# ViacheslavDanilov/oct_segmentation

Hardware: AMD Instinct MI355X
Metric: OCT frames/sec (704x704, bf16) fwd+bwd (higher is better)
Workload: dtype bf16; 1 GPU; unetplusplus/resnet101 1-class 704x704, batch 16/GPU, fwd+Dice+bwd+allreduce+Adam; global_batch=16, parallelism=dp1

## Files before the change

### oct_segmentation_amd/csrc/conv_mfma.hip

```cpp
#include "common.h"
#include "conv_common.h"
#include "kernels.h"

#include <type_traits>

namespace octseg {

#ifdef OCTSEG_STAMP
#define STAMP(var) do { __builtin_amdgcn_sched_barrier(0); asm volatile("s_memtime %0\n\ts_waitcnt lgkmcnt(0)" : "=s"(var) :: "memory"); __builtin_amdgcn_sched_barrier(0); } while (0)
#else
#define STAMP(var) do { } while (0)
#endif

struct RowMap {
  static constexpr unsigned MASK_B = 0xF00F0FF0u;
  static __device__ __forceinline__ int ty(int rr) { return (MASK_B >> rr) & 1; }
  static __device__ __forceinline__ int tx(int rr) {
    const unsigned grp = ((MASK_B >> rr) & 1) ? MASK_B : ~MASK_B;
    return __popc(grp & ((1u << rr) - 1u));
  }
};

static constexpr int wave_mt(int NT, int RB) { return (NT == 4 && RB == 64) ? 4 : 2; }

// ... 271 lines not shown
          const int gy = y0 + ty, gx = x0 + tx;
          float val = acc16[mb][nb][j] + bias;
          if (a.relu_out) val = clamp_lo(val, 0.f);
          if (cok && pv && gy < a.OH && gx < a.OW) {
            s1[nb] += val; s2[nb] += val * val;
            if (head) {
              const DstDesc& d = a.dst[0];
              const int oy = gy * a.ostride + a.ooy, ox = gx * a.ostride + a.oox;
              ((float*)d.ptr)[(((size_t)n * a.Cout + co) * d.H + oy) * d.W + ox] = val;
            }
          }
          if (!head) *(unsigned short*)(otile + prow * OPITCH + cl * 2) = Tr<T>::bits16(val);
        }
    }
  } else
#pragma unroll
  for (int nt = 0; nt < NT; ++nt) {
    s1[nt] = 0.f; s2[nt] = 0.f;
    const int cl = wn * NT * 32 + nt * 32 + r;
    const int co = co0 + cl;
    const bool cok = co < a.Cout;
    const float bias = (a.bias != nullptr && cok) ? a.bias[co] : 0.f;
#pragma unroll
    for (int mt = 0; mt < MT; ++mt) {
#pragma unroll
      for (int i = 0; i < 16; ++i) {
        const int rr = (i & 3) + 8 * (i >> 2) + 4 * h;
        const int ty = wm * 2 * MT + mt * 2 + RowMap::ty(rr), tx = RowMap::tx(rr);
        const int gy = y0 + ty, gx = x0 + tx;
        float val = acc[mt][nt][i] + bias;
        if (a.relu_out) val = clamp_lo(val, 0.f);
        if (cok && gy < a.OH && gx < a.OW) {
          s1[nt] += val; s2[nt] += val * val;
          if (head) {
            const DstDesc& d = a.dst[0];
            const int oy = gy * a.ostride + a.ooy, ox = gx * a.ostride + a.oox;
            ((float*)d.ptr)[(((size_t)n * a.Cout + co) * d.H + oy) * d.W + ox] = val;
          }
        }
        if (!head) {
          if (sizeof(T) == 4) *(float*)(otile + (ty * TW + tx) * OPITCH + cl * 4) = val;
          else *(unsigned short*)(otile + (ty * TW + tx) * OPITCH + cl * 2) = Tr<T>::bits16(val);
        }
      }
    }
  }
  if (a.stat_slab != nullptr) {
    if constexpr (M16) {
#pragma unroll
      for (int nb = 0; nb < NCB; ++nb) {
        s1[nb] += __shfl_xor(s1[nb], 16); s1[nb] += __shfl_xor(s1[nb], 32);
        s2[nb] += __shfl_xor(s2[nb], 16); s2[nb] += __shfl_xor(s2[nb], 32);
        if (g16 == 0) {
          const int cl = wn * NT * 32 + nb * 16 + r16;
          red[(wm * BN + cl) * 2 + 0] = s1[nb];
          red[(wm * BN + cl) * 2 + 1] = s2[nb];
        }
      }
    } else
#pragma unroll
    for (int nt = 0; nt < NT; ++nt) {
      s1[nt] += __shfl_xor(s1[nt], 32);
      s2[nt] += __shfl_xor(s2[nt], 32);
      if (h == 0) {
        const int cl = wn * NT * 32 + nt * 32 + r;
        red[(wm * BN + cl) * 2 + 0] = s1[nt];
        red[(wm * BN + cl) * 2 + 1] = s2[nt];
      }
    }
  }
  __syncthreads();
  if (a.stat_slab != nullptr && tid < BN) {
    const int co = co0 + tid;
    if (co < a.Cout) {
      float t1 = 0.f, t2 = 0.f;
#pragma unroll
      for (int w = 0; w < WM; ++w) { t1 += red[(w * BN + tid) * 2]; t2 += red[(w * BN + tid) * 2 + 1]; }
      float* slab = a.stat_slab + ((size_t)(a.slab_row0 + (w_mt)) * a.Cout + co) * 2;
      slab[0] = t1; slab[1] = t2;
    }
  }
  if (!head) {
    for (int v = tid; v < BM * OVPR; v += NTHREADS) {
      const int p = v / OVPR, cvv = v % OVPR;
      int ty = p >> 4, tx = p & 15;
      if constexpr (T11) { if (p >= 121) continue; ty = p / 11; tx = p - ty * 11; }
      const int gy = y0 + ty, gx = x0 + tx;
      const int co = co0 + cvv * VEC;
      if (gy >= a.OH || gx >= a.OW || co >= a.Cout) continue;
      char* dptr = (char*)a.dst[0].ptr; int dC = a.dst[0].C, dc0 = a.dst[0].c0, dH = a.dst[0].H, dW = a.dst[0].W, dacc = a.dst[0].accum;
      int dpool = a.dst[0].pool;
#pragma unroll
      for (int i = 1; i < MAX_SRC; ++i)
        if (i < a.ndst && co >= a.dst[i].c0) {
          dptr = (char*)a.dst[i].ptr; dC = a.dst[i].C; dc0 = a.dst[i].c0; dH = a.dst[i].H; dW = a.dst[i].W; dacc = a.dst[i].accum;
          dpool = a.dst[i].pool;
        }
      if (dpool) {
        if ((ty | tx) & 1) continue;
        const char* l0 = otile + p * OPITCH + cvv * 16;
        const uint4 q[4] = {*(const uint4*)l0, *(const uint4*)(l0 + OPITCH), *(const uint4*)(l0 + TW * OPITCH),
                            *(const uint4*)(l0 + (TW + 1) * OPITCH)};
        uint4* gq = (uint4*)(dptr + ((((size_t)n * dH + (gy >> 1)) * dW + (gx >> 1)) * dC + (co - dc0)) * sizeof(T));
        uint4 old = make_uint4(0, 0, 0, 0);
        if (dacc) old = *gq;
        unsigned o[4] = {old.x, old.y, old.z, old.w}, r4[4];
        const unsigned* qq[4] = {&q[0].x, &q[1].x, &q[2].x, &q[3].x};
#pragma unroll
        for (int i = 0; i < 4; ++i) {
          if (sizeof(T) == 4) {
            float sacc = dacc ? __uint_as_float(o[i]) : 0.f;
#pragma unroll
            for (int j = 0; j < 4; ++j) sacc += __uint_as_float(qq[j][i]);
            r4[i] = __float_as_uint(sacc);
          } else {
            float lo = dacc ? Tr<T>::lo(o[i]) : 0.f, hi = dacc ? Tr<T>::hi(o[i]) : 0.f;
#pragma unroll
            for (int j = 0; j < 4; ++j) { lo += Tr<T>::lo(qq[j][i]); hi += Tr<T>::hi(qq[j][i]); }
            r4[i] = Tr<T>::pk(lo, hi);
          }
        }
        *gq = make_uint4(r4[0], r4[1], r4[2], r4[3]);
        continue;
      }
      const int oy = gy * a.ostride + a.ooy, ox = gx * a.ostride + a.oox;
      uint4* gp = (uint4*)(dptr + ((((size_t)n * dH + oy) * dW + ox) * dC + (co - dc0)) * sizeof(T));
      uint4 val = *(const uint4*)(otile + p * OPITCH + cvv * 16);
      if (a.out_mode == OUT_ACCUM || dacc) {
        const uint4 old = *gp;
        if (sizeof(T) == 4) {
          val.x = __float_as_uint(__uint_as_float(val.x) + __uint_as_float(old.x));
          val.y = __float_as_uint(__uint_as_float(val.y) + __uint_as_float(old.y));
          val.z = __float_as_uint(__uint_as_float(val.z) + __uint_as_float(old.z));
          val.w = __float_as_uint(__uint_as_float(val.w) + __uint_as_float(old.w));
        } else {
          unsigned nv[4] = {val.x, val.y, val.z, val.w};
          const unsigned ov[4] = {old.x, old.y, old.z, old.w};
#pragma unroll
          for (int i = 0; i < 4; ++i) {
            const float lo = Tr<T>::lo(nv[i]) + Tr<T>::lo(ov[i]);
            const float hi = Tr<T>::hi(nv[i]) + Tr<T>::hi(ov[i]);
            nv[i] = Tr<T>::pk(lo, hi);
          }
          val = make_uint4(nv[0], nv[1], nv[2], nv[3]);
        }
      }
      *gp = val;
    }
  }
}

template <int RB> struct ConvCfg { static constexpr int PITCH = RB + 16, KSTEPS = RB / 32, VPR = RB / 16; };

enum { LOOP_GENERIC = 0, LOOP_RESIDENT = 1, LOOP_1X1 = 2, LOOP_RUN9 = 3, LOOP_RUN9S = 4, LOOP_MASKED = 5, LOOP_T11 = 6, LOOP_MASKED_T11 = 7 };

template <typename T, int NT, int WN, int WM, int RB, int LOOP>
__global__ __launch_bounds__(64 * WM * WN, ((WM * WN == 4 && wave_mt(NT, RB) == 2) ? 2 : 1)) void conv_mfma_kernel(const ConvArgs a, const int mode) {
  constexpr int MT = wave_mt(NT, RB);
  const int dbuf = mode & 1;
  constexpr bool resident = LOOP == LOOP_RESIDENT;
  extern __shared__ __attribute__((aligned(16))) char smem[];
  constexpr int NTHREADS = 64 * WM * WN;
  constexpr int BN = NT * 32 * WN;
  constexpr int TH = 2 * MT * WM;
  constexpr int KC = RB / (int)sizeof(T);
  constexpr int PITCH = ConvCfg<RB>::PITCH, KSTEPS = ConvCfg<RB>::KSTEPS, VPR = ConvCfg<RB>::VPR;
  constexpr int NWAVES = WM * WN;
  constexpr int BBYTES = BN * RB;
  constexpr int NDMA = BBYTES / 1024;
  constexpr int DPW = (NDMA + NWAVES - 1) / NWAVES;
  constexpr int SWZ_DIV = 256 / RB;
  constexpr int MAXP = 4;
  typedef WindowStager<T, RB, NTHREADS> Stager;

#ifdef OCTSEG_STAMP
  unsigned long long k0 = 0, k1 = 0, k2 = 0, k3 = 0;
  STAMP(k0);
#endif
  const int tid = threadIdx.x, lane = tid & 63, wave = tid >> 6;
  const int wm = wave / WN, wn = wave % WN;
  const int r = lane & 31, h = lane >> 5;

  constexpr bool T11 = LOOP == LOOP_T11 || LOOP == LOOP_MASKED_T11;
  const TilePos tp = map_tile<TH, BN, T11>(a);
  const int n = tp.n, y0 = tp.y0, x0 = tp.x0, nt_idx = tp.nt_idx;

  const bool single = a.ntaps == 1;
  const int lstride = single ? 1 : a.istride;
  const int smul = single ? a.istride : 1;
  constexpr int THe = T11 ? 11 : TH, TWe = T11 ? 11 : TW;
  const int RH = single ? THe : (THe - 1) * a.istride + a.span_y;
  const int RW = single ? TWe : (TWe - 1) * a.istride + a.span_x;
  const int npix = RH * RW;
  const int npass = (npix + Stager::PSTEP - 1) / Stager::PSTEP;
  const float inv_rw = 1.0f / (float)RW;
  const int gy0 = y0 * a.istride + a.min_dy, gx0 = x0 * a.istride + a.min_dx;

  const int abytes = npass * Stager::PSTEP * PITCH;
  char* ldsA = smem;
  char* ldsB = smem + (dbuf ? 2 : 1) * abytes;

  constexpr bool M16 = conv_m16<T>(MT);
  f32x16_t acc[M16 ? 1 : MT][M16 ? 1 : NT];
#pragma unroll
  for (int i = 0; i < (M16 ? 1 : MT); ++i)
#pragma unroll
    for (int j = 0; j < (M16 ? 1 : NT); ++j)
#pragma unroll
      for (int k = 0; k < 16; ++k) acc[i][j][k] = 0.f;
  f32x4_t acc16[M16 ? 2 * MT : 1][M16 ? 2 * NT : 1];
#pragma unroll
  for (int i = 0; i < (M16 ? 2 * MT : 1); ++i)
#pragma unroll
    for (int j = 0; j < (M16 ? 2 * NT : 1); ++j)
#pragma unroll
      for (int k = 0; k < 4; ++k) acc16[i][j][k] = 0.f;
  const int r16 = lane & 15, g16 = lane >> 4;
  int abase16[2 * MT], bbase16[2 * NT], bswz16[2 * NT];
#pragma unroll
  for (int mb = 0; mb < 2 * MT; ++mb) {
    abase16[mb] = (((wm * 2 * MT + mb) * lstride) * RW + r16 * lstride) * PITCH + g16 * 16;
    if constexpr (T11) {
      const int p = min((wm * 2 * MT + mb) * 16 + r16, 120);
      const int pty = p / 11;
      abase16[mb] = (pty * RW + (p - pty * 11)) * PITCH + g16 * 16;
    }
  }
#pragma unroll
  for (int nb = 0; nb < 2 * NT; ++nb) {
    const int row = wn * NT * 32 + nb * 16 + r16;
    bbase16[nb] = row * RB;
    bswz16[nb] = (row / SWZ_DIV) & (VPR - 1);
  }

  int abase[MT], bbase[NT];
#pragma unroll
  for (int mt = 0; mt < MT; ++mt) {
    const int ty = wm * 2 * MT + mt * 2 + RowMap::ty(r), tx = RowMap::tx(r);
    abase[mt] = ((ty * lstride) * RW + tx * lstride) * PITCH + h * 16;
  }
  int bswz[NT];
#pragma unroll
  for (int nt = 0; nt < NT; ++nt) {
    const int row = wn * NT * 32 + nt * 32 + r;
    bbase[nt] = row * RB;
    bswz[nt] = (row / SWZ_DIV) & (VPR - 1);
  }

  const int nchunks = (a.Cin + KC - 1) / KC;
  const char* Wp = (const char*)a.W;

  const int ntiles_n = gridDim.y;
  const int wave_u = __builtin_amdgcn_readfirstlane(wave);
  const unsigned ldsB_addr = (unsigned)(size_t)(__attribute__((address_space(3))) char*)ldsB;
  const char* dma_src0 = Wp + (size_t)nt_idx * BBYTES + (size_t)wave_u * DPW * 1024 + lane * 16;
  const size_t slab_stride = (size_t)ntiles_n * BBYTES;
  const bool dma_wave = NDMA % NWAVES == 0 || wave_u * DPW < NDMA;
  auto dmaB = [&](int slab_idx, int slot) {
    if (dma_wave) {
      const char* gsrc0 = dma_src0 + (size_t)slab_idx * slab_stride;
#pragma unroll
      for (int j = 0; j < DPW; ++j) {
        const char* gsrc = gsrc0 + j * 1024;
        const unsigned dst = __builtin_amdgcn_readfirstlane(ldsB_addr + slot * BBYTES + (wave_u * DPW + j) * 1024);
        unsigned keep;
        asm volatile("s_mov_b32 %0, m0\n\ts_mov_b32 m0, %2\n\ts_nop 0\n\tglobal_load_lds_dwordx4 %1, off\n\ts_mov_b32 m0, %0"
                     : "=&s"(keep) : "v"(gsrc), "s"(dst) : "memory");
      }
    }
  };
  int v_toff = 0, v_tapw = 0;
  if (lane < a.ntaps) {
    v_toff = single ? 0 : ((a.tap_dy[lane] - a.min_dy) * RW + (a.tap_dx[lane] - a.min_dx)) * PITCH;
    v_tapw = a.tap_w[lane];
  }
  auto stage_full = [&](const Stager& sg, char* dst) {
    for (int p = 0; p < npass; p += MAXP) {
      uint4 v[MAXP];
      bool ok[MAXP];
#pragma unroll
      for (int u = 0; u < MAXP; ++u) v[u] = sg.load(min(p + u, npass - 1), n, gy0, gx0, smul, RW, npix, inv_rw, a.IH, a.IW, ok[u]);
#pragma unroll
      for (int u = 0; u < MAXP; ++u) sg.write(dst, min(p + u, npass - 1), v[u], ok[u]);
    }
  };
  auto mma_tap = [&](const char* awin, const char* bsl, int toff) {
    if constexpr (M16) {
      constexpr int KQ = RB / 64;
      uint4 fa[2 * MT], fb[KQ][2 * NT];
      auto ldA = [&](int mb, int kq) __attribute__((always_inline)) { fa[mb] = *(const uint4*)(awin + abase16[mb] + toff + kq * 64); };
      auto ldB = [&](int kq, int nb) __attribute__((always_inline)) {
        fb[kq][nb] = *(const uint4*)(bsl + bbase16[nb] + (((kq * 4 + g16) ^ bswz16[nb]) * 16));
      };
      ldA(0, 0);
#pragma unroll
      for (int nb = 0; nb < 2 * NT; ++nb) ldB(0, nb);
#pragma unroll
      for (int mb = 1; mb < 2 * MT; ++mb) ldA(mb, 0);
#pragma unroll
      for (int kq = 0; kq < KQ; ++kq)
#pragma unroll
        for (int mb = 0; mb < 2 * MT; ++mb) {
          __builtin_amdgcn_sched_barrier(0);
#pragma unroll
          for (int nb = 0; nb < 2 * NT; ++nb) Tr<T>::mma16(fa[mb], fb[kq][nb], acc16[mb][nb]);
          if (kq + 1 < KQ) {
            ldA(mb, kq + 1);
// ... 43 lines not shown
#pragma unroll
      for (int kq = 0; kq < KQ; ++kq)
#pragma unroll
        for (int mb = 0; mb < 2 * MT; ++mb) {
          __builtin_amdgcn_sched_barrier(0);
#pragma unroll
          for (int nb = 0; nb < 2 * NT; ++nb) Tr<T>::mma16(fa[mb], fb[kq][nb], acc16[mb][nb]);
          if (kq + 1 < KQ) {
            ldA(mb, kq + 1);
#pragma unroll
            for (int nb = 0; nb < 2 * NT; ++nb)
              if (nb * 2 * MT / (2 * NT) == mb) ldB(kq + 1, nb);
          }
          __builtin_amdgcn_sched_barrier(0);
          {
            constexpr int NSTEP = KQ * 2 * MT;
            const int step = kq * 2 * MT + mb;
            if (step == NSTEP / 4 - 1 || (NSTEP < 4 && step == 0)) f0();
            if (step == NSTEP / 2 - 1) f1();
            if (step == (3 * NSTEP) / 4 - 1 || (NSTEP < 4 && step == NSTEP - 1)) f2();
            __builtin_amdgcn_sched_barrier(0);
          }
        }
    } else {
    constexpr int NFB = KSTEPS >= 3 ? 3 : KSTEPS;
    uint4 af[NFB][MT], bf[NFB][NT];
    auto frag_load = [&](int buf, int ks) {
#pragma unroll
      for (int mt = 0; mt < MT; ++mt) af[buf][mt] = *(const uint4*)(awin + abase[mt] + toff + ks * 32);
#pragma unroll
      for (int nt = 0; nt < NT; ++nt) bf[buf][nt] = *(const uint4*)(bsl + bbase[nt] + (((ks * 2 + h) ^ bswz[nt]) * 16));
    };
    frag_load(0, 0);
    if (KSTEPS > 1) frag_load(1, 1);
#pragma unroll
    for (int ks = 0; ks < KSTEPS; ++ks) {
      if (ks + 2 < KSTEPS) frag_load((ks + 2) % NFB, ks + 2);
      __builtin_amdgcn_sched_barrier(0);
#pragma unroll
      for (int mt = 0; mt < MT; ++mt)
#pragma unroll
        for (int nt = 0; nt < NT; ++nt) Tr<T>::mma(af[ks % NFB][mt], bf[ks % NFB][nt], acc[mt][nt]);
      __builtin_amdgcn_sched_barrier(0);
      if (ks == 0) f0();
      if (ks == 1) f1();
      if (ks == 2 || (KSTEPS == 2 && ks == 1)) f2();
      __builtin_amdgcn_sched_barrier(0);
    }
    }
  };

  {
    Stager cur;
    cur.setup(a.src, a.nsrc, a.Cin, 0, tid);
    if (resident) {
      for (int t = 0; t < a.ntaps; ++t) dmaB(a.tap_w[t] * nchunks, t);
    } else if constexpr (LOOP == LOOP_MASKED || LOOP == LOOP_MASKED_T11) {
      dmaB(a.tap_w[a.src_taps[0] & 15] * nchunks, 0);
    } else {
      dmaB(a.tap_w[0] * nchunks, 0);
      if constexpr (LOOP == LOOP_RUN9 || LOOP == LOOP_RUN9S) dmaB(a.tap_w[1] * nchunks, 1);
    }
    stage_full(cur, ldsA);
  }
  asm volatile("s_waitcnt vmcnt(0)" ::: "memory");
  __syncthreads();
#ifdef OCTSEG_STAMP
  STAMP(k1);
#endif

#ifdef OCTSEG_STAMP
  unsigned long long tsum[6] = {0, 0, 0, 0, 0, 0};
#endif
  const int IHl = a.IH, IWl = a.IW, ntaps = a.ntaps;
  const int p0w = tid / VPR;
  const int hy_first = (int)(((float)p0w + 0.5f) * inv_rw), hx_first = p0w - hy_first * RW;
  const int dq = Stager::PSTEP / RW, dr = Stager::PSTEP - dq * RW;
  auto run = [&](auto ppt_c, auto dbuf_c) {
    constexpr int PPT = decltype(ppt_c)::value;
    constexpr bool DBUF = decltype(dbuf_c)::value;
    int it = 0;
    int tap2 = ntaps == 1 ? 0 : 1, chunk2 = ntaps == 1 ? min(1, nchunks - 1) : 0;
    for (int chunk = 0; chunk < nchunks; ++chunk) {
      const bool has_next = chunk + 1 < nchunks;
      Stager nxt;
      nxt.setup(a.src, a.nsrc, a.Cin, has_next ? chunk + 1 : chunk, tid, a.src_uniform != 0);
      nxt.bind_image(n);
      const char* awin = ldsA + ((DBUF && (chunk & 1)) ? abytes : 0);
      char* anext = ldsA + ((chunk & 1) ? 0 : abytes);
      int hy = hy_first, hx = hx_first, hp = p0w;
      char* wrow = anext + p0w * PITCH;
      for (int t = 0; t < ntaps; ++t, ++it) {
        unsigned long long s0 = 0, s1 = 0, s2 = 0, s3 = 0, s4 = 0, s5 = 0;
        (void)s0; (void)s1; (void)s2; (void)s3; (void)s4; (void)s5;
        STAMP(s0);
        uint4 av[PPT];
        bool aok[PPT];
        char* wr[PPT];
        if constexpr (DBUF) {
#pragma unroll
          for (int u = 0; u < PPT; ++u) {
            av[u] = nxt.load_at(hy, hx, hp < npix, gy0, gx0, smul, IHl, IWl, aok[u]);
            wr[u] = wrow;
            const bool adv = hp + Stager::PSTEP < npass * Stager::PSTEP;
            if (adv) {
              hp += Stager::PSTEP; wrow += Stager::PSTEP * PITCH;
              hy += dq; hx += dr;
              if (hx >= RW) { hx -= RW; hy += 1; }
            }
          }
        }
        dmaB(__builtin_amdgcn_readlane(v_tapw, tap2) * nchunks + chunk2, (it + 1) & 1);
        const int toff = __builtin_amdgcn_readlane(v_toff, t);
        STAMP(s1);
        mma_tap(awin, ldsB + (it & 1) * BBYTES, toff);
        STAMP(s2);
        __builtin_amdgcn_sched_barrier(0);
        if constexpr (DBUF) {
#pragma unroll
          for (int u = 0; u < PPT; ++u) nxt.write_at(wr[u], av[u], aok[u]);
        }
        STAMP(s3);
        asm volatile("s_waitcnt vmcnt(0)" ::: "memory");
        asm volatile("s_waitcnt lgkmcnt(0)" ::: "memory");
        STAMP(s4);
        __builtin_amdgcn_s_barrier();
        asm volatile("" ::: "memory");
        STAMP(s5);
#ifdef OCTSEG_STAMP
        tsum[0] += s1 - s0; tsum[1] += s2 - s1; tsum[2] += s3 - s2; tsum[3] += s4 - s3; tsum[4] += s5 - s4; tsum[5] += 1;
#endif
        if (++tap2 == ntaps) { tap2 = 0; chunk2 = min(chunk2 + 1, nchunks - 1); }
      }
      if constexpr (!DBUF) {
        if (has_next) {
          stage_full(nxt, ldsA);
          __syncthreads();
        }
      }
    }
  };
  auto run_t11 = [&](auto np_c) {
    constexpr int NP = decltype(np_c)::value;
    int it = 0;
    int tap2 = 1, chunk2 = 0;
    for (int chunk = 0; chunk < nchunks; ++chunk) {
      const bool has_next = chunk + 1 < nchunks;
      Stager nxt;
      nxt.setup(a.src, a.nsrc, a.Cin, has_next ? chunk + 1 : chunk, tid, a.src_uniform != 0);
      nxt.bind_image(n);
      uint4 av[NP];
      bool aok[NP];
      int hy = hy_first, hx = hx_first, hp = p0w;
#pragma unroll
      for (int t = 0; t < 9; ++t, ++it) {
        if (t < NP) {
          av[t] = nxt.load_at(hy, hx, hp < npix, gy0, gx0, smul, IHl, IWl, aok[t]);
          const bool adv = hp + Stager::PSTEP < npass * Stager::PSTEP;
          if (adv) {
            hp += Stager::PSTEP;
            hy += dq; hx += dr;
            if (hx >= RW) { hx -= RW; hy += 1; }
          }
        }
        dmaB(__builtin_amdgcn_readlane(v_tapw, tap2) * nchunks + chunk2, (it + 1) & 1);
        const int toff = __builtin_amdgcn_readlane(v_toff, t);
        mma_tap(ldsA, ldsB + (it & 1) * BBYTES, toff);
        __builtin_amdgcn_sched_barrier(0);
        asm volatile("s_waitcnt vmcnt(0)" ::: "memory");
        asm volatile("s_waitcnt lgkmcnt(0)" ::: "memory");
        __builtin_amdgcn_s_barrier();
        asm volatile("" ::: "memory");
        if (++tap2 == 9) { tap2 = 0; chunk2 = min(chunk2 + 1, nchunks - 1); }
      }
      if (has_next) {
#pragma unroll
        for (int u = 0; u < NP; ++u)
          if (u < npass) nxt.write_at(ldsA + (p0w + u * Stager::PSTEP) * PITCH, av[u], aok[u]);
        __syncthreads();
      }
    }
  };
  auto run_masked = [&](auto ppt_c) {
    constexpr int PPT = decltype(ppt_c)::value;
    const int tps = a.taps_per_src;
    auto list_of = [&](int chunk) -> int {
      int l = a.src_taps[0];
#pragma unroll
      for (int i = 1; i < MAX_SRC; ++i)
        if (i < a.nsrc && chunk * KC >= a.src[i].c0) l = a.src_taps[i];
      return l;
    };
    int it = 0;
    for (int chunk = 0; chunk < nchunks; ++chunk) {
      const bool has_next = chunk + 1 < nchunks;
      const int cnext = has_next ? chunk + 1 : chunk;
      Stager nxt;
      nxt.setup(a.src, a.nsrc, a.Cin, cnext, tid, a.src_uniform != 0);
      nxt.bind_image(n);
      const char* awin = ldsA + ((chunk & 1) ? abytes : 0);
      char* anext = ldsA + ((chunk & 1) ? 0 : abytes);
      const int lst = list_of(chunk), lst_n = list_of(cnext);
      int hy = hy_first, hx = hx_first, hp = p0w;
      char* wrow = anext + p0w * PITCH;
      for (int k = 0; k < tps; ++k, ++it) {
        const int t = (lst >> (4 * k)) & 15;
        uint4 av[PPT];
        bool aok[PPT];
        char* wr[PPT];
        const bool same = k + 1 < tps;
        const int tn = same ? (lst >> (4 * (k + 1))) & 15 : lst_n & 15;
        const int toff = __builtin_amdgcn_readlane(v_toff, t);
        mma_tap_f(awin, ldsB + (it & 1) * BBYTES, toff,
          [&]() {
            dmaB(__builtin_amdgcn_readlane(v_tapw, tn) * nchunks + (same ? chunk : cnext), (it + 1) & 1);
#pragma unroll
            for (int u = 0; u < PPT; ++u) {
              av[u] = nxt.load_at(hy, hx, hp < npix, gy0, gx0, smul, IHl, IWl, aok[u]);
              wr[u] = wrow;
              const bool adv = hp + Stager::PSTEP < npass * Stager::PSTEP;
              if (adv) {
                hp += Stager::PSTEP; wrow += Stager::PSTEP * PITCH;
                hy += dq; hx += dr;
                if (hx >= RW) { hx -= RW; hy += 1; }
              }
            }
          },
          [&]() {},
          [&]() {
#pragma unroll
            for (int u = 0; u < PPT; ++u) nxt.write_at(wr[u], av[u], aok[u]);
          });
        __builtin_amdgcn_sched_barrier(0);
        asm volatile("s_waitcnt vmcnt(0)" ::: "memory");
        asm volatile("s_waitcnt lgkmcnt(0)" ::: "memory");
        __builtin_amdgcn_s_barrier();
        asm volatile("" ::: "memory");
      }
    }
  };
  typedef __attribute__((ext_vector_type(4))) unsigned u32x4_t;
  auto run1p = [&]() __attribute__((always_inline)) {
    constexpr int PPT = 4;
    constexpr int NQ = 2 * (Stager::VEC / 4);
    constexpr int NLD = PPT + NQ;
    constexpr int NDM = NDMA % NWAVES == 0 ? DPW : 0;
    Stager sA, sB;
    u32x4_t avA0 = {0, 0, 0, 0}, avA1 = avA0, avA2 = avA0, avA3 = avA0, qA0 = avA0, qA1 = avA0, qA2 = avA0, qA3 = avA0;
    u32x4_t avB0 = avA0, avB1 = avA0, avB2 = avA0, avB3 = avA0, qB0 = avA0, qB1 = avA0, qB2 = avA0, qB3 = avA0;
    bool okA[PPT], okB[PPT];
    int pyc[PPT], pxc[PPT];
    bool pok[PPT];
    {
      int hy = hy_first, hx = hx_first, hp = p0w;
#pragma unroll
      for (int u = 0; u < PPT; ++u) {
        const int iy = gy0 + hy * smul, ix = gx0 + hx * smul;
        pok[u] = hp < npix && (unsigned)iy < (unsigned)IHl && (unsigned)ix < (unsigned)IWl;
        pyc[u] = min(max(iy, 0), IHl - 1); pxc[u] = min(max(ix, 0), IWl - 1);
        const bool adv = hp + Stager::PSTEP < npass * Stager::PSTEP;
        if (adv) {
          hp += Stager::PSTEP;
          hy += dq; hx += dr;
          if (hx >= RW) { hx -= RW; hy += 1; }
        }
      }
    }
    const bool usrc = a.src_uniform != 0;
#define OCTSEG_LD4(dst, ptr) asm volatile("global_load_dwordx4 %0, %1, off" : "=v"(dst) : "v"(ptr))
#define OCTSEG_LD4_16(dst, ptr) asm volatile("global_load_dwordx4 %0, %1, off offset:16" : "=v"(dst) : "v"(ptr))
    auto load_chunk = [&](Stager& sg, int chunk, u32x4_t& v0, u32x4_t& v1, u32x4_t& v2, u32x4_t& v3, u32x4_t& q0, u32x4_t& q1,
                          u32x4_t& q2, u32x4_t& q3, bool (&ok)[PPT]) __attribute__((always_inline)) {
      sg.select(a.src, a.nsrc, a.Cin, min(chunk, nchunks - 1), tid, usrc);
      sg.bind_image(n);
      const char* scp = sg.has_aff ? (const char*)(sg.s.scale + sg.s.cl) : Wp;
      const char* shp = sg.has_aff ? (const char*)(sg.s.shift + sg.s.cl) : Wp;
      OCTSEG_LD4(q0, scp);
      if constexpr (Stager::VEC == 8) OCTSEG_LD4_16(q1, scp);
      OCTSEG_LD4(q2, shp);
      if constexpr (Stager::VEC == 8) OCTSEG_LD4_16(q3, shp);
      const char* g0 = sg.addr_xy(pyc[0], pxc[0]); OCTSEG_LD4(v0, g0);
      const char* g1 = sg.addr_xy(pyc[1], pxc[1]); OCTSEG_LD4(v1, g1);
      const char* g2 = sg.addr_xy(pyc[2], pxc[2]); OCTSEG_LD4(v2, g2);
      const char* g3 = sg.addr_xy(pyc[3], pxc[3]); OCTSEG_LD4(v3, g3);
#pragma unroll
      for (int u = 0; u < PPT; ++u) ok[u] = sg.cvalid && pok[u];
    };
    auto body = [&](int c, Stager& sld, u32x4_t& l0, u32x4_t& l1, u32x4_t& l2, u32x4_t& l3, u32x4_t& lq0, u32x4_t& lq1, u32x4_t& lq2,
                    u32x4_t& lq3, bool (&okl)[PPT], Stager& sst, u32x4_t& s0, u32x4_t& s1, u32x4_t& s2, u32x4_t& s3, u32x4_t& sq0,
                    u32x4_t& sq1, u32x4_t& sq2, u32x4_t& sq3, const bool (&oks)[PPT]) __attribute__((always_inline)) {
      char* wnext = ldsA + ((c & 1) ? 0 : abytes);
      auto row = [&](int u) { return wnext + (min(u, npass - 1) * Stager::PSTEP + p0w) * PITCH; };
      mma_tap_f(ldsA + ((c & 1) ? abytes : 0), ldsB + (c & 1) * BBYTES, 0,
        [&]() {
          dmaB(a.tap_w[0] * nchunks + min(c + 1, nchunks - 1), (c + 1) & 1);
          load_chunk(sld, c + 2, l0, l1, l2, l3, lq0, lq1, lq2, lq3, okl);
        },
        [&]() {
          asm volatile("s_waitcnt vmcnt(%8)" : "+v"(s0), "+v"(s1), "+v"(s2), "+v"(s3), "+v"(sq0), "+v"(sq1), "+v"(sq2), "+v"(sq3)
                       : "n"(NDM + NLD) : "memory");
#pragma unroll
          for (int i = 0; i < 4; ++i) {
            sst.sc[i] = __uint_as_float(sq0[i]); sst.sh[i] = __uint_as_float(sq2[i]);
            if constexpr (Stager::VEC == 8) { sst.sc[4 + i] = __uint_as_float(sq1[i]); sst.sh[4 + i] = __uint_as_float(sq3[i]); }
          }
          sst.write_at(row(0), __builtin_bit_cast(uint4, s0), oks[0]);
          sst.write_at(row(1), __builtin_bit_cast(uint4, s1), oks[1]);
        },
        [&]() {
          sst.write_at(row(2), __builtin_bit_cast(uint4, s2), oks[2]);
// ... 71 lines not shown
                if (hx >= RW) { hx -= RW; hy += 1; }
              }
            }
          },
          [&]() {
            STAMP(s2);
            if constexpr (TT >= 1) {
              if constexpr ((TT - 1) & 1) {
                asm volatile("s_waitcnt vmcnt(%1)" : "+v"(avB) : "n"(DPW + W) : "memory");
                STAMP(s3);
                wv = nxt.prep(__builtin_bit_cast(uint4, avB), okB);
              } else {
                asm volatile("s_waitcnt vmcnt(%1)" : "+v"(avA) : "n"(DPW + W) : "memory");
                STAMP(s3);
                wv = nxt.prep(__builtin_bit_cast(uint4, avA), okA);
              }
            } else {
              asm volatile("s_waitcnt vmcnt(%4)" : "+v"(q0), "+v"(q1), "+v"(q2), "+v"(q3) : "n"(DPW + W) : "memory");
              STAMP(s3);
#pragma unroll
              for (int i = 0; i < 4; ++i) {
                nxt.sc[i] = __uint_as_float(q0[i]); nxt.sh[i] = __uint_as_float(q2[i]);
                if constexpr (Stager::VEC == 8) { nxt.sc[4 + i] = __uint_as_float(q1[i]); nxt.sh[4 + i] = __uint_as_float(q3[i]); }
              }
            }
#ifdef OCTSEG_STAMP
            tsum[2] += s3 - s2;
#endif
          },
          [&]() {
            if constexpr (TT >= 1) *(uint4*)((((TT - 1) & 1) ? wrB : wrA) + nxt.cv * 16) = wv;
          });
        __builtin_amdgcn_sched_barrier(0);
        unsigned long long s2e = 0; (void)s2e;
        STAMP(s2e);
        asm volatile("s_waitcnt lgkmcnt(0)" ::: "memory");
        STAMP(s4);
        __builtin_amdgcn_s_barrier();
        asm volatile("" ::: "memory");
        STAMP(s5);
#ifdef OCTSEG_STAMP
        tsum[0] += s1 - s0; tsum[1] += s2e - s1; tsum[3] += s4 - s2e; tsum[4] += s5 - s4; tsum[5] += 1;
#endif
        if (++tap2 == 9) { tap2 = 0; chunk2 = min(chunk2 + 1, nchunks - 1); }
      };
      tap(std::integral_constant<int, 0>{}); tap(std::integral_constant<int, 1>{}); tap(std::integral_constant<int, 2>{});
      tap(std::integral_constant<int, 3>{}); tap(std::integral_constant<int, 4>{}); tap(std::integral_constant<int, 5>{});
      tap(std::integral_constant<int, 6>{}); tap(std::integral_constant<int, 7>{}); tap(std::integral_constant<int, 8>{});
    }
    asm volatile("s_waitcnt vmcnt(0)" ::: "memory");
    __syncthreads();
  };
  auto run_masked_rp = [&]() {
    constexpr int NP = 6, TPS = 4;
    auto list_of = [&](int chunk) -> int {
      if (a.taps_per_src == 0) return 0x3210;
      int l = a.src_taps[0];
#pragma unroll
      for (int i = 1; i < MAX_SRC; ++i)
        if (i < a.nsrc && chunk * KC >= a.src[i].c0) l = a.src_taps[i];
      return l;
    };
    int it = 0;
    for (int chunk = 0; chunk < nchunks; ++chunk) {
      const bool has_next = chunk + 1 < nchunks;
      const int cnext = has_next ? chunk + 1 : chunk;
      Stager nxt;
      nxt.setup(a.src, a.nsrc, a.Cin, cnext, tid, a.src_uniform != 0);
      nxt.bind_image(n);
      const int lst = list_of(chunk), lst_n = list_of(cnext);
      uint4 av[NP];
      bool aok[NP];
      int hy = hy_first, hx = hx_first, hp = p0w;
      auto load_pass = [&](auto uc) __attribute__((always_inline)) {
        constexpr int U = decltype(uc)::value;
        av[U] = nxt.load_at(hy, hx, hp < npix, gy0, gx0, smul, IHl, IWl, aok[U]);
        const bool adv = hp + Stager::PSTEP < npass * Stager::PSTEP;
        if (adv) {
          hp += Stager::PSTEP;
          hy += dq; hx += dr;
          if (hx >= RW) { hx -= RW; hy += 1; }
        }
      };
      auto tap = [&](auto kc) __attribute__((always_inline)) {
        constexpr int K = decltype(kc)::value;
        const int t = (lst >> (4 * K)) & 15;
        if constexpr (K == 0) { load_pass(std::integral_constant<int, 0>{}); load_pass(std::integral_constant<int, 1>{}); }
        if constexpr (K == 1) { load_pass(std::integral_constant<int, 2>{}); load_pass(std::integral_constant<int, 3>{}); }
        if constexpr (K == 2) load_pass(std::integral_constant<int, 4>{});
        if constexpr (K == 3) load_pass(std::integral_constant<int, 5>{});
        const bool same = K + 1 < TPS;
        const int tn = same ? (lst >> (4 * (K + 1))) & 15 : lst_n & 15;
        dmaB(__builtin_amdgcn_readlane(v_tapw, tn) * nchunks + (same ? chunk : cnext), (it + 1) & 1);
        const int toff = __builtin_amdgcn_readlane(v_toff, t);
        mma_tap(ldsA, ldsB + (it & 1) * BBYTES, toff);
        __builtin_amdgcn_sched_barrier(0);
        asm volatile("s_waitcnt vmcnt(0)" ::: "memory");
        asm volatile("s_waitcnt lgkmcnt(0)" ::: "memory");
        __builtin_amdgcn_s_barrier();
        asm volatile("" ::: "memory");
        ++it;
      };
      tap(std::integral_constant<int, 0>{}); tap(std::integral_constant<int, 1>{});
      tap(std::integral_constant<int, 2>{}); tap(std::integral_constant<int, 3>{});
      if (has_next) {
#pragma unroll
        for (int u = 0; u < NP; ++u)
          if (u < npass) nxt.write_at(ldsA + (p0w + u * Stager::PSTEP) * PITCH, av[u], aok[u]);
        __syncthreads();
      }
    }
  };
  if constexpr (LOOP == LOOP_RESIDENT) {
    for (int t = 0; t < ntaps; ++t) mma_tap(ldsA, ldsB + t * BBYTES, __builtin_amdgcn_readlane(v_toff, t));
    __syncthreads();
  } else if constexpr (LOOP == LOOP_RUN9S) {
    if constexpr (NDMA % NWAVES == 0 && RB == 128) {
      int slotC = 0, slotS = 2;
      auto tap = [&](auto tc) __attribute__((always_inline)) {
        constexpr int TT = decltype(tc)::value;
        const int toff = __builtin_amdgcn_readlane(v_toff, TT);
        const char* bsl = ldsB + slotC * BBYTES;
        if (++slotC == 3) slotC = 0;
        mma_tap_f(ldsA, bsl, toff,
          [&]() {
            if constexpr (TT + 2 < 9) dmaB(__builtin_amdgcn_readlane(v_tapw, TT + 2) * nchunks, slotS);
            if (++slotS == 3) slotS = 0;
          },
          [&]() {
            if constexpr (TT + 2 < 9) asm volatile("s_waitcnt vmcnt(%0)" :: "n"(DPW) : "memory");
            else asm volatile("s_waitcnt vmcnt(0)" ::: "memory");
          },
          [&]() {});
        __builtin_amdgcn_sched_barrier(0);
        asm volatile("s_waitcnt lgkmcnt(0)" ::: "memory");
        __builtin_amdgcn_s_barrier();
        asm volatile("" ::: "memory");
      };
      tap(std::integral_constant<int, 0>{}); tap(std::integral_constant<int, 1>{}); tap(std::integral_constant<int, 2>{});
      tap(std::integral_constant<int, 3>{}); tap(std::integral_constant<int, 4>{}); tap(std::integral_constant<int, 5>{});
      tap(std::integral_constant<int, 6>{}); tap(std::integral_constant<int, 7>{}); tap(std::integral_constant<int, 8>{});
    }
  } else if constexpr (LOOP == LOOP_RUN9) {
    if constexpr (NDMA % NWAVES == 0 && (RB == 128 || (RB == 64 && NT == 4))) run9r();
  } else if constexpr (LOOP == LOOP_MASKED_T11) {
    run_masked_rp();
  } else if constexpr (LOOP == LOOP_MASKED) {
    if constexpr (WM == 2) { if (dbuf) run_masked(std::integral_constant<int, 2>{}); else run_masked_rp(); }
    else run_masked(std::integral_constant<int, 2>{});
  } else if constexpr (LOOP == LOOP_1X1) {
    run1p();
  } else if constexpr (LOOP == LOOP_T11) {
    run_t11(std::integral_constant<int, 6>{});
  } else {
    if (dbuf) run(std::integral_constant<int, 1>{}, std::true_type{});
    else run(std::integral_constant<int, 1>{}, std::false_type{});
  }

#ifdef OCTSEG_STAMP
  STAMP(k2);
#endif
  conv_epilogue<T, NT, WN, WM, MT, T11>(a, smem, acc, acc16, tp);
#ifdef OCTSEG_STAMP
  STAMP(k3);
  if (a.stamp != nullptr && lane == 0) {
    for (int i = 0; i < 6; ++i) atomicAdd(a.stamp + i, tsum[i]);
    atomicAdd(a.stamp + 8, k1 - k0); atomicAdd(a.stamp + 9, k2 - k1); atomicAdd(a.stamp + 10, k3 - k2); atomicAdd(a.stamp + 11, 1ull);
  }
#endif
}

namespace {

struct Variant { int NT, WN, WM, RB; };

size_t variant_lds(const ConvArgs& a, const Variant& v, int esz, int dbuf, int* npass_out) {
  const int TH = 2 * wave_mt(v.NT, v.RB) * v.WM, BN = v.NT * 32 * v.WN, BM = TH * TW, PITCH = v.RB + 16;
  (void)PITCH;
  const bool single = a.ntaps == 1;
  const int RH = single ? TH : (TH - 1) * a.istride + a.span_y;
  const int RW = single ? TW : (TW - 1) * a.istride + a.span_x;
  const int npix = RH * RW;
  const int nthreads = 64 * v.WM * v.WN;
  const int pstep = nthreads / (v.RB / 16);
  if (npass_out) *npass_out = (npix + pstep - 1) / pstep;
  const int npass = (npix + pstep - 1) / pstep;
  const size_t abytes = (size_t)npass * pstep * PITCH;
  const size_t main_loop = (dbuf ? 2 : 1) * abytes + 2 * (size_t)BN * v.RB;
  const size_t epi = (size_t)BM * (BN * esz + 16) + (size_t)v.WM * BN * 2 * sizeof(float);
  return main_loop > epi ? main_loop : epi;
}

template <typename T, int NT, int WN, int WM, int RB, int LOOP>
hipError_t launch_loop(const ConvArgs& a, int mode, size_t lds, hipStream_t st) {
  constexpr int BN = NT * 32 * WN, TH = 2 * wave_mt(NT, RB) * WM;
  const int mtiles = (LOOP == LOOP_T11 || LOOP == LOOP_MASKED_T11) ? a.N * (a.OH / 11) * (a.OW / 11) : a.N * ((a.OH + TH - 1) / TH) * ((a.OW + TW - 1) / TW);
  dim3 grid(mtiles, (a.Cout + BN - 1) / BN);
  static bool attr_set = false;
  if (!attr_set) {
    hipError_t e = hipFuncSetAttribute((const void*)conv_mfma_kernel<T, NT, WN, WM, RB, LOOP>,
                                       hipFuncAttributeMaxDynamicSharedMemorySize, 160 * 1024);
    if (e != hipSuccess) return e;
    attr_set = true;
  }
  hipLaunchKernelGGL((conv_mfma_kernel<T, NT, WN, WM, RB, LOOP>), grid, dim3(64 * WM * WN), lds, st, a, mode);
  return hipGetLastError();
}

template <typename T, int NT, int WN, int WM, int RB>
hipError_t launch_variant(const ConvArgs& a, int mode, int loop, size_t lds, hipStream_t st) {
  switch (loop) {
    case LOOP_RESIDENT: return launch_loop<T, NT, WN, WM, RB, LOOP_RESIDENT>(a, mode, lds, st);
    case LOOP_1X1: return launch_loop<T, NT, WN, WM, RB, LOOP_1X1>(a, mode, lds, st);
    case LOOP_RUN9:
      if constexpr ((RB == 128 || (RB == 64 && NT == 4)) && ((NT * 32 * WN * RB / 1024) % (WM * WN)) == 0) return launch_loop<T, NT, WN, WM, RB, LOOP_RUN9>(a, mode, lds, st);
      else return hipErrorInvalidValue;
    case LOOP_RUN9S:
      if constexpr (RB == 128 && ((NT * 32 * WN * RB / 1024) % (WM * WN)) == 0) return launch_loop<T, NT, WN, WM, RB, LOOP_RUN9S>(a, mode, lds, st);
      else return hipErrorInvalidValue;
    case LOOP_MASKED:
      if constexpr (RB == 128 && sizeof(T) == 2 && NT == 2) return launch_loop<T, NT, WN, WM, RB, LOOP_MASKED>(a, mode, lds, st);
      else return hipErrorInvalidValue;
    case LOOP_MASKED_T11:
      if constexpr (RB == 128 && sizeof(T) == 2 && NT == 2 && WN == 2 && WM == 2) return launch_loop<T, NT, WN, WM, RB, LOOP_MASKED_T11>(a, mode, lds, st);
      else return hipErrorInvalidValue;
    case LOOP_T11:
      if constexpr (RB == 128 && sizeof(T) == 2 && NT == 2 && WN == 2 && WM == 2) return launch_loop<T, NT, WN, WM, RB, LOOP_T11>(a, mode, lds, st);
      else return hipErrorInvalidValue;
    default: return launch_loop<T, NT, WN, WM, RB, LOOP_GENERIC>(a, mode, lds, st);
  }
}

struct Choice { Variant v; int dbuf; size_t lds; int resident; int ring3; int ring1; int tile11; };

static bool tile11_geom(const ConvArgs& a, int esz) {
  if (esz != 2 || a.taps_per_src > 0) return false;
  if (a.ntaps != 9 || a.span_x != 3 || a.span_y != 3 || a.istride != 1 || a.ostride != 1 || a.ooy != 0 || a.oox != 0) return false;
  if (a.out_mode == OUT_HEAD_NCHW || a.IH != a.OH || a.IW != a.OW || a.OH % 11 != 0 || a.OW % 11 != 0 || a.OH > 88 || a.OW > 88) return false;
  if (a.OH % 16 == 0 && a.OW % 16 == 0) return false;
  if (a.Cout <= 64 || a.Cin < 64) return false;
  const long long wg16 = (long long)a.N * ((a.OH + 15) / 16) * ((a.OW + 15) / 16) * ((a.Cout + 127) / 128);
  static const long long minwg = getenv("OCTSEG_TILE11_MINWG") ? atoll(getenv("OCTSEG_TILE11_MINWG")) : 256;
  const long long wg11 = (long long)a.N * (a.OH / 11) * (a.OW / 11) * ((a.Cout + 127) / 128);
  return wg16 <= 4608 && wg11 >= minwg;
}

static size_t lds_single128(int esz) {
  const size_t main_loop = (size_t)6 * 32 * 144 + 2 * (size_t)128 * 128;
  const size_t epi = (size_t)128 * (128 * esz + 16) + (size_t)2 * 128 * 2 * sizeof(float);
  return main_loop > epi ? main_loop : epi;
}

static bool any_pooled_dst(const ConvArgs& a) {
  for (int i = 0; i < a.ndst; ++i)
    if (a.dst[i].pool != 0) return true;
  return false;
}

static Choice choose(const ConvArgs& a, int esz) {
  Choice c;
  c.ring3 = 0; c.ring1 = 0; c.tile11 = 0;
  const bool t11 = tile11_geom(a, esz);
  if (t11 && !any_pooled_dst(a)) {
    c.v = Variant{2, 2, 2, 128}; c.dbuf = 0; c.resident = 0; c.tile11 = 1; c.lds = lds_single128(esz);
    return c;
  }
  if (esz == 2 && a.taps_per_src == 0 && a.ntaps == 4 && a.span_x == 2 && a.span_y == 2 && a.istride == 1 &&
      a.out_mode != OUT_HEAD_NCHW && a.Cout > 64 && a.Cin >= 64) {
    c.v = Variant{2, 2, 2, 128}; c.dbuf = 0; c.resident = 0; c.tile11 = 3;
    c.lds = lds_single128(esz);
    return c;
  }
  if (a.taps_per_src > 0) {
    static const bool force_dbuf = getenv("OCTSEG_MASKED_DBUF") != nullptr;
    if (!force_dbuf && a.taps_per_src == 4 && esz == 2 && a.ntaps == 9 && a.span_x == 3 && a.span_y == 3) {
      c.v = Variant{2, 2, 2, 128}; c.dbuf = 0; c.resident = 0;
      c.tile11 = (!any_pooled_dst(a) && a.OH % 11 == 0 && a.OW % 11 == 0 && !(a.OH % 16 == 0 && a.OW % 16 == 0) && a.OH <= 88 && a.OW <= 88) ? 1 : 0;
      c.lds = lds_single128(esz);
      return c;
    }
    for (int wm = 4; wm >= 2; wm -= 2) {
      const Variant v{2, 2, wm, 128};
      int npass = 0;
      const size_t lds = variant_lds(a, v, esz, 1, &npass);
      if (lds <= (size_t)160 * 1024 && npass <= 2 * a.taps_per_src) { c.v = v; c.dbuf = 1; c.lds = lds; c.resident = 0; return c; }
    }
    c.v = Variant{2, 2, 2, 128}; c.dbuf = 1; c.resident = 0; c.lds = (size_t)1 << 30;
    return c;
  }
  {
    const int n256 = (a.Cout + 255) / 256;
    const int kc = 64 / esz;
    const bool p3 = esz == 2 && a.ostride == 1 && a.OH % 16 == 0 && a.OW % 16 == 0 && a.IH == a.OH && a.IW == a.OW;
    const bool fits = !p3 && a.Cout == 256 && a.Cin >= 256 && (long long)a.N * ((a.OH + 15) / 16) * ((a.OW + TW - 1) / TW) >= 1024;
    if (!t11 && fits && a.ntaps == 9 && a.istride == 1 && a.Cout > 128 && (n256 * 256 - a.Cout) * 10 <= a.Cout && a.Cin > kc) {
      const Variant v{4, 2, 2, 64};
      int npass = 0;
      const size_t lds = variant_lds(a, v, esz, 1, &npass);
      const size_t slab = (size_t)256 * 64;
      const long long wgs = (long long)a.N * ((a.OH + 15) / 16) * ((a.OW + TW - 1) / TW) * n256;
      if (wgs >= 384 && npass <= 8 && lds + slab <= (size_t)160 * 1024) {
        c.v = v; c.dbuf = 1; c.lds = lds + slab; c.resident = 0; c.ring3 = 1;
        return c;
      }
    }
  }
  int NT, WN;
  if (a.Cout > 64) { NT = 2; WN = 2; } else if (a.Cout > 32) { NT = 1; WN = 2; } else { NT = 1; WN = 1; }
  {
    const int t128 = (a.Cout + 127) / 128;
    if (a.Cout > 64 && a.ntaps == 9 && a.Cin <= 128 / esz && a.Cout % 64 == 0 && (t128 * 128 - a.Cout) * 4 >= t128 * 128) { NT = 1; WN = 2; }
  }
  bool small_grid = false;
  {
    const int bn = NT * 32 * WN;
    const long long w16 = (long long)a.N * ((a.OH + 15) / 16) * ((a.OW + TW - 1) / TW) * ((a.Cout + bn - 1) / bn);
    small_grid = a.ntaps > 1 && w16 < 128;
    if (small_grid && a.Cout > 64) { NT = 1; WN = 2; }
  }
  const int kc128 = 128 / esz;
  const int RB = a.Cin <= kc128 / 2 ? 64 : 128;
  auto util = [&](int TH) {
    const double ty = (a.OH + TH - 1) / TH, tx = (a.OW + TW - 1) / TW;
    return (double)a.OH * a.OW / (ty * TH * tx * TW);
  };
  const size_t cap = 160 * 1024;
  int wm_first = util(8) > 1.15 * util(16) ? 2 : 4;
  {
    const int kc = (a.Cin <= (128 / esz) / 2 ? 64 : 128) / esz;
    if ((a.ntaps == 1 || a.Cin <= kc) && WN > 1) wm_first = 2;
    if (a.ntaps == 9 && a.Cin <= kc && a.Cout <= 64 && WN > 1) wm_first = 4;
    if (a.ntaps == 9 && a.Cin > kc && WN == 2 && NT == 1) wm_first = 2;
    if (a.ntaps == 9 && a.Cin > kc) {
      const int BN = NT * 32 * WN;
      const long long b16 = (long long)a.N * ((a.OH + 15) / 16) * ((a.OW + TW - 1) / TW) * ((a.Cout + BN - 1) / BN);
      const long long b8 = (long long)a.N * ((a.OH + 7) / 8) * ((a.OW + TW - 1) / TW) * ((a.Cout + BN - 1) / BN);
      if (b16 <= 256 && b8 > 256) wm_first = 4;
    }
  }
  if (small_grid) wm_first = 2;
  const int order[2] = {wm_first, wm_first == 4 ? 2 : 4};
  const int nchunks_c = (a.Cin + RB / esz - 1) / (RB / esz);
  for (int pref_dbuf = nchunks_c > 1 ? 1 : 0; pref_dbuf >= 0; --pref_dbuf)
    for (int k = 0; k < 2; ++k) {
      Variant v{NT, WN, order[k], RB};
      int npass = 0;
      const size_t lds = variant_lds(a, v, esz, pref_dbuf, &npass);
      const bool fits_pipe = a.ntaps == 1 ? npass <= 4 : npass <= a.ntaps;
      if (lds <= cap && (!pref_dbuf || fits_pipe)) {
        c.v = v; c.dbuf = pref_dbuf; c.lds = lds; c.resident = 0;
        {
          const size_t slab = (size_t)v.NT * 32 * v.WN * v.RB;
          const int nd = (int)(slab / 1024), nw = v.WM * v.WN;
          if (pref_dbuf && a.ntaps == 9 && npass <= 8 && nd % nw == 0 && lds + slab <= cap) { c.ring3 = 1; c.lds = lds + slab; }
        }
        const size_t slab = (size_t)v.NT * 32 * v.WN * v.RB;
        if (nchunks_c == 1 && a.ntaps > 1 && a.ntaps * slab <= 40 * 1024) {
          const size_t extra = (size_t)(a.ntaps - 2) * slab;
          if (lds + extra <= 64 * 1024) { c.resident = 1; c.lds = lds + extra; }
        }
        {
          const int nd = (int)(slab / 1024), nw = v.WM * v.WN;
          if (!c.resident && !pref_dbuf && nchunks_c == 1 && a.ntaps == 9 && v.RB == 128 && nd % nw == 0 && lds + slab <= cap) {
            c.ring1 = 1; c.lds = lds + slab;
          }
        }
        return c;
      }
    }
  c.v = Variant{NT, WN, 2, RB}; c.dbuf = 0; c.resident = 0; c.lds = variant_lds(a, c.v, esz, 0, nullptr);
  return c;
}

template <typename T>
hipError_t dispatch(const ConvArgs& a_in, hipStream_t st) {
  const Choice c = choose(a_in, (int)sizeof(T));
  if (c.lds > 160 * 1024) return hipErrorInvalidValue;
  const Variant& v = c.v;
  ConvArgs a = a_in;
  {
    const int KC = v.RB / (int)sizeof(T);
    a.src_uniform = 1;
    for (int i = 1; i < a.nsrc; ++i)
      if (a.src[i].c0 % KC != 0) a.src_uniform = 0;
  }
  const int loop = a.taps_per_src > 0 ? (c.tile11 ? LOOP_MASKED_T11 : LOOP_MASKED) : c.tile11 == 3 ? LOOP_MASKED : c.tile11 ? LOOP_T11
                   : c.resident ? LOOP_RESIDENT : (c.ring3 ? LOOP_RUN9 : (c.ring1 ? LOOP_RUN9S : ((a.ntaps == 1 && c.dbuf) ? LOOP_1X1 : LOOP_GENERIC)));
#define OCTSEG_CASE(NT_, WN_, WM_, RB_)                                             \
  if (v.NT == NT_ && v.WN == WN_ && v.WM == WM_ && v.RB == RB_)                     \
    return launch_variant<T, NT_, WN_, WM_, RB_>(a, c.dbuf, loop, c.lds, st);
  OCTSEG_CASE(4, 2, 2, 64)
  OCTSEG_CASE(2, 2, 4, 128)
  OCTSEG_CASE(2, 2, 2, 128)
  OCTSEG_CASE(1, 2, 4, 128)
  OCTSEG_CASE(1, 2, 2, 128)
  OCTSEG_CASE(1, 1, 4, 128)
  OCTSEG_CASE(1, 1, 2, 128)
  OCTSEG_CASE(2, 2, 4, 64)
  OCTSEG_CASE(2, 2, 2, 64)
  OCTSEG_CASE(1, 2, 4, 64)
  OCTSEG_CASE(1, 2, 2, 64)
  OCTSEG_CASE(1, 1, 4, 64)
  OCTSEG_CASE(1, 1, 2, 64)
#undef OCTSEG_CASE
  return hipErrorInvalidValue;
}

}

ConvPackInfo conv_pack_info(const ConvArgs& a, int dtype) {
  const Choice c = choose(a, (int)dtype_size(dtype));
  ConvPackInfo p;
  p.BN = c.v.NT * 32 * c.v.WN;
  p.RB = c.v.RB;
  const int KC = p.RB / (int)dtype_size(dtype);
  p.nchunks = (a.Cin + KC - 1) / KC;
  p.ntiles = (a.Cout + p.BN - 1) / p.BN;
  return p;
}

int conv_num_mtiles(const ConvArgs& a, int dtype) {
  const Choice c = choose(a, (int)dtype_size(dtype));
  if (c.tile11 == 1) return a.N * (a.OH / 11) * (a.OW / 11);
  const int TH = 2 * wave_mt(c.v.NT, c.v.RB) * c.v.WM;
  return a.N * ((a.OH + TH - 1) / TH) * ((a.OW + TW - 1) / TW);
}

static bool flatten_1x1(ConvArgs& a) {
  if (a.ntaps != 1 || a.istride != 1 || a.ostride != 1 || a.out_mode == OUT_HEAD_NCHW) return false;
  if (a.tap_dy[0] != 0 || a.tap_dx[0] != 0) return false;
  const long long npix = (long long)a.N * a.OH * a.OW;
  if (npix % TW != 0 || a.IH != a.OH || a.IW != a.OW) return false;
  for (int i = 0; i < a.nsrc; ++i)
    if (a.src[i].up || a.src[i].H != a.IH || a.src[i].W != a.IW) return false;
  for (int i = 0; i < a.ndst; ++i)
    if (a.dst[i].H != a.OH || a.dst[i].W != a.OW) return false;
  const int rows = (int)(npix / TW);
  a.N = 1; a.IH = a.OH = rows; a.IW = a.OW = TW;
  for (int i = 0; i < a.nsrc; ++i) { a.src[i].H = rows; a.src[i].W = TW; }
  for (int i = 0; i < a.ndst; ++i) { a.dst[i].H = rows; a.dst[i].W = TW; }
  return true;
}

ConvRoute conv_route(const ConvArgs& a, int dtype) {
  if (a.taps_per_src > 0) return ROUTE_MFMA;
  if (thin_conv_eligible(a, dtype)) return ROUTE_THIN;
  if (gemm1x1_eligible(a, dtype)) return ROUTE_GEMM1X1;
  if (conv3x3p_eligible(a, dtype)) return ROUTE_CONV3X3P;
  return ROUTE_MFMA;
}

int conv_mfma_tile(const ConvArgs& a0, int dtype) {
  ConvArgs a = a0;
  if (a.taps_per_src == 0) flatten_1x1(a);
  const Choice c = choose(a, (int)dtype_size(dtype));
  return c.tile11 == 1 ? TILE_11 : c.v.NT == 4 ? TILE_WIDE_N : TILE_16;
}

int conv_num_mtiles_flat(const ConvArgs& a0, int dtype) {
  switch (conv_route(a0, dtype)) {
    case ROUTE_THIN: return thin_conv_rows(a0);
    case ROUTE_GEMM1X1: return gemm1x1_rows(a0);
    case ROUTE_CONV3X3P: return conv3x3p_rows(a0);
    case ROUTE_MFMA: break;
  }
  ConvArgs a = a0;
  flatten_1x1(a);
  return conv_num_mtiles(a, dtype);
}

bool conv_masked_eligible(const ConvArgs& a, int dtype) {
  if (dtype == DT_F32 || a.taps_per_src <= 0 || a.taps_per_src > 8 || a.ntaps < 2 || a.ntaps > 16) return false;
  if (a.istride != 1 || a.ostride != 1 || a.out_mode == OUT_HEAD_NCHW || a.Cout <= 64 || a.Cout % 8 != 0) return false;
  const int KC = 64;
  for (int i = 0; i < a.nsrc; ++i)
    if (a.src[i].c0 % KC != 0 || a.src[i].up) return false;
  if (a.Cin % KC != 0) return false;
  const Choice c = choose(a, (int)dtype_size(dtype));
  return c.lds <= (size_t)160 * 1024;
}

hipError_t launch_conv(int dtype, const ConvArgs& a0, hipStream_t st) {
  if (a0.ntaps <= 0) return hipSuccess;
  switch (conv_route(a0, dtype)) {
    case ROUTE_THIN: return launch_thin_conv(dtype, a0, st);
    case ROUTE_GEMM1X1: return launch_gemm1x1(dtype, a0, st);
    case ROUTE_CONV3X3P: return launch_conv3x3p(dtype, a0, st);
    case ROUTE_MFMA: break;
  }
  if (a0.taps_per_src > 0) {
    if (!conv_masked_eligible(a0, dtype)) return hipErrorInvalidValue;
    ConvArgs a = a0;
    a.tile_order = 1;
    return dtype == DT_F16 ? dispatch<f16_t>(a, st) : dispatch<bf16_t>(a, st);
  }
  ConvArgs a = a0;
  flatten_1x1(a);
  {
    int wt = 0;
    for (int t = 0; t < a.ntaps; ++t) wt = a.tap_w[t] + 1 > wt ? a.tap_w[t] + 1 : wt;
    const size_t wbytes = (size_t)wt * a.Cout * a.Cin * dtype_size(dtype);
    static const int force = getenv("OCTSEG_TILE_ORDER") ? atoi(getenv("OCTSEG_TILE_ORDER")) : -1;
    (void)wbytes;
    a.tile_order = force >= 0 ? force : 1;
  }
  if (dtype == DT_F32) return dispatch<float>(a, st);
  if (dtype == DT_F16) return dispatch<f16_t>(a, st);
  return dispatch<bf16_t>(a, st);
}

}
```

Measured before the change: 255.3 frames/s.

## Add RUN9P conv loop with 2x1x4 tile for 64-wide 3x3 convs

Adds a new loop variant that reuses the per-tap pipelined t11 loop with up to 11 prefetch passes, spreading A-tile loads across the nine taps instead of front-loading them. The heuristic sends stride-1 3x3 convs with Cin above one chunk and a 64-wide N tile to a new NT=2, WN=1, WM=4, RB=128 configuration, which is tall in M and narrow in N. This is meant to improve overlap of global loads with MFMA work and to change the tile shape for these layers, at the cost of another template instantiation and more register pressure from the larger prefetch array.

```diff
diff --git a/oct_segmentation_amd/csrc/conv_mfma.hip b/oct_segmentation_amd/csrc/conv_mfma.hip
--- a/oct_segmentation_amd/csrc/conv_mfma.hip
+++ b/oct_segmentation_amd/csrc/conv_mfma.hip
@@ -447,7 +447,7 @@
 
 template <int RB> struct ConvCfg { static constexpr int PITCH = RB + 16, KSTEPS = RB / 32, VPR = RB / 16; };
 
-enum { LOOP_GENERIC = 0, LOOP_RESIDENT = 1, LOOP_1X1 = 2, LOOP_RUN9 = 3, LOOP_RUN9S = 4, LOOP_MASKED = 5, LOOP_T11 = 6, LOOP_MASKED_T11 = 7 };
+enum { LOOP_GENERIC = 0, LOOP_RESIDENT = 1, LOOP_1X1 = 2, LOOP_RUN9 = 3, LOOP_RUN9S = 4, LOOP_MASKED = 5, LOOP_T11 = 6, LOOP_MASKED_T11 = 7, LOOP_RUN9P = 8 };
 
 template <typename T, int NT, int WN, int WM, int RB, int LOOP>
 __global__ __launch_bounds__(64 * WM * WN, ((WM * WN == 4 && wave_mt(NT, RB) == 2) ? 2 : 1)) void conv_mfma_kernel(const ConvArgs a, const int mode) {
@@ -797,10 +797,12 @@
       uint4 av[NP];
       bool aok[NP];
       int hy = hy_first, hx = hx_first, hp = p0w;
+      int pi = 0;
 #pragma unroll
       for (int t = 0; t < 9; ++t, ++it) {
-        if (t < NP) {
-          av[t] = nxt.load_at(hy, hx, hp < npix, gy0, gx0, smul, IHl, IWl, aok[t]);
+#pragma unroll
+        for (int u = 0; u < (NP + 8 - t) / 9; ++u, ++pi) {
+          av[pi] = nxt.load_at(hy, hx, hp < npix, gy0, gx0, smul, IHl, IWl, aok[pi]);
           const bool adv = hp + Stager::PSTEP < npass * Stager::PSTEP;
           if (adv) {
             hp += Stager::PSTEP;
@@ -1178,6 +1180,8 @@
     run1p();
   } else if constexpr (LOOP == LOOP_T11) {
     run_t11(std::integral_constant<int, 6>{});
+  } else if constexpr (LOOP == LOOP_RUN9P) {
+    run_t11(std::integral_constant<int, 11>{});
   } else {
     if (dbuf) run(std::integral_constant<int, 1>{}, std::true_type{});
     else run(std::integral_constant<int, 1>{}, std::false_type{});
@@ -1235,7 +1239,14 @@
 
 template <typename T, int NT, int WN, int WM, int RB>
 hipError_t launch_variant(const ConvArgs& a, int mode, int loop, size_t lds, hipStream_t st) {
+  if constexpr (NT == 2 && WN == 1) {
+    if constexpr (sizeof(T) == 2 && WM == 4 && RB == 128) {
+      if (loop == LOOP_RUN9P) return launch_loop<T, NT, WN, WM, RB, LOOP_RUN9P>(a, mode, lds, st);
+    }
+    return hipErrorInvalidValue;
+  } else
   switch (loop) {
+    case LOOP_RUN9P: return hipErrorInvalidValue;
     case LOOP_RESIDENT: return launch_loop<T, NT, WN, WM, RB, LOOP_RESIDENT>(a, mode, lds, st);
     case LOOP_1X1: return launch_loop<T, NT, WN, WM, RB, LOOP_1X1>(a, mode, lds, st);
     case LOOP_RUN9:
@@ -1257,7 +1268,7 @@
   }
 }
 
-struct Choice { Variant v; int dbuf; size_t lds; int resident; int ring3; int ring1; int tile11; };
+struct Choice { Variant v; int dbuf; size_t lds; int resident; int ring3; int ring1; int tile11; int rp11; };
 
 static bool tile11_geom(const ConvArgs& a, int esz) {
   if (esz != 2 || a.taps_per_src > 0) return false;
@@ -1285,7 +1296,7 @@
 
 static Choice choose(const ConvArgs& a, int esz) {
   Choice c;
-  c.ring3 = 0; c.ring1 = 0; c.tile11 = 0;
+  c.ring3 = 0; c.ring1 = 0; c.tile11 = 0; c.rp11 = 0;
   const bool t11 = tile11_geom(a, esz);
   if (t11 && !any_pooled_dst(a)) {
     c.v = Variant{2, 2, 2, 128}; c.dbuf = 0; c.resident = 0; c.tile11 = 1; c.lds = lds_single128(esz);
@@ -1337,6 +1348,7 @@
     const int t128 = (a.Cout + 127) / 128;
     if (a.Cout > 64 && a.ntaps == 9 && a.Cin <= 128 / esz && a.Cout % 64 == 0 && (t128 * 128 - a.Cout) * 4 >= t128 * 128) { NT = 1; WN = 2; }
   }
+  const bool n64 = NT == 1 && WN == 2;
   bool small_grid = false;
   {
     const int bn = NT * 32 * WN;
@@ -1346,6 +1358,13 @@
   }
   const int kc128 = 128 / esz;
   const int RB = a.Cin <= kc128 / 2 ? 64 : 128;
+  if (n64 && esz == 2 && a.Cin > kc128 && a.ntaps == 9 && a.span_x == 3 && a.span_y == 3 && a.istride == 1 && a.ostride == 1 && a.ooy == 0 && a.oox == 0 &&
+      a.out_mode != OUT_HEAD_NCHW) {
+    const Variant v{2, 1, 4, 128};
+    int npass = 0;
+    const size_t lds = variant_lds(a, v, esz, 0, &npass);
+    if (npass <= 11) { c.v = v; c.dbuf = 0; c.resident = 0; c.rp11 = 1; c.lds = lds; return c; }
+  }
   auto util = [&](int TH) {
     const double ty = (a.OH + TH - 1) / TH, tx = (a.OW + TW - 1) / TW;
     return (double)a.OH * a.OW / (ty * TH * tx * TW);
@@ -1411,13 +1430,14 @@
       if (a.src[i].c0 % KC != 0) a.src_uniform = 0;
   }
   const int loop = a.taps_per_src > 0 ? (c.tile11 ? LOOP_MASKED_T11 : LOOP_MASKED) : c.tile11 == 3 ? LOOP_MASKED : c.tile11 ? LOOP_T11
-                   : c.resident ? LOOP_RESIDENT : (c.ring3 ? LOOP_RUN9 : (c.ring1 ? LOOP_RUN9S : ((a.ntaps == 1 && c.dbuf) ? LOOP_1X1 : LOOP_GENERIC)));
+                   : c.rp11 ? LOOP_RUN9P : c.resident ? LOOP_RESIDENT : (c.ring3 ? LOOP_RUN9 : (c.ring1 ? LOOP_RUN9S : ((a.ntaps == 1 && c.dbuf) ? LOOP_1X1 : LOOP_GENERIC)));
 #define OCTSEG_CASE(NT_, WN_, WM_, RB_)                                             \
   if (v.NT == NT_ && v.WN == WN_ && v.WM == WM_ && v.RB == RB_)                     \
     return launch_variant<T, NT_, WN_, WM_, RB_>(a, c.dbuf, loop, c.lds, st);
   OCTSEG_CASE(4, 2, 2, 64)
   OCTSEG_CASE(2, 2, 4, 128)
   OCTSEG_CASE(2, 2, 2, 128)
+  OCTSEG_CASE(2, 1, 4, 128)
   OCTSEG_CASE(1, 2, 4, 128)
   OCTSEG_CASE(1, 2, 2, 128)
   OCTSEG_CASE(1, 1, 4, 128)
```

New measurement: 258.3 frames/s, median of 6. 1.01x the previous value.
